# Cameronr11/GAN-Variant-Research

Hardware: AMD Instinct MI355X
Metric: images/sec (G+D train step) 256x256 CUT (higher is better)
Workload: dtype bf16; 1 GPU; CUT ResNet-9 G + PatchGAN D + PatchNCE + identity + lazy R1 + DiffAugment, 256x256, batch 16 per GPU (BASELINE.json configs[2]); global_batch=16, parallelism=dp1

## Files before the change

### gan-variant-research_amd/csrc/wgrad_patch.hip

```cpp
#include <stdlib.h>
#include <atomic>
#include "common.h"

namespace {

constexpr int KM = 128;
constexpr int NB = 128, CB = 64;
constexpr int RX = 320;
constexpr int GT_BYTES = KM * 256, XP_BYTES = RX * 128, STAGE_BYTES = GT_BYTES + XP_BYTES;
constexpr int LDS_BYTES = 2 * STAGE_BYTES;
constexpr int NT = 9;
constexpr int RING_SLOTS = 4, RING_PITCH = 136;
constexpr int LDS_BYTES_RING = 2 * GT_BYTES + RING_SLOTS * RING_PITCH * 128;

struct WpArgs {
  const char* x; const char* g; float* part;
  int B, HoWo, Wo, lgWo, spi, per;
  int ipb;
  int Cx, N, pitch, nrows;
  int x_Hp, x_Wp, x_y0, x_x0;
  int g_Hp, g_Wp, g_C, g_y0, g_x0;
  int NBLK, CBLK;
};

__device__ __forceinline__ void glds16q(const char* gbase, uint32_t goff, char* lds) {
  __builtin_amdgcn_global_load_lds((const __attribute__((address_space(1))) void*)(gbase + goff),
                                   (__attribute__((address_space(3))) void*)lds, 16, 0, 0);
}

template <bool RING>
__global__ __launch_bounds__(512) void wgrad_patch_kernel(WpArgs a) {
  extern __shared__ __attribute__((aligned(1024))) char lds[];
  const int tid = threadIdx.x, lane = tid & 63, wave = tid >> 6;

  int bid = (gridDim.x & 7) == 0 ? (int)(blockIdx.x & 7) * (int)(gridDim.x >> 3) + (int)(blockIdx.x >> 3) : (int)blockIdx.x;
  const int cb = bid % a.CBLK; bid /= a.CBLK;
  const int nb = bid % a.NBLK; bid /= a.NBLK;
  const int sp = bid;
  const int b0 = a.ipb > 1 ? sp * a.ipb : sp / a.spi, sub = a.ipb > 1 ? 0 : sp - b0 * a.spi;
  const int m_begin = sub * a.per, m_end = min(a.HoWo, m_begin + a.per);
  const int nst_img = (m_end - m_begin + KM - 1) / KM;
  const int nstage = nst_img * a.ipb;
  const int n0 = nb * NB, c0 = cb * CB;

  const int gr = tid >> 4, gp = tid & 15;
  const uint32_t gsrc = (uint32_t)((n0 + ((gp ^ ((gr & 7) << 1)) << 3)) * 2);
  const int xr = tid >> 3, xp = tid & 7;
  const uint32_t xsrc = (uint32_t)((c0 + ((((xp >> 1) ^ ((xr >> 1) & 3)) << 1 | (xp & 1)) << 3)) * 2);
  const uint32_t x_pixb = (uint32_t)a.Cx * 2u, g_pixb = (uint32_t)a.g_C * 2u;

  char* const ring = lds + 2 * GT_BYTES;
  const uint32_t ring_rowb = (uint32_t)(a.pitch * 128);
  const int b = b0;
  auto load_row = [&](int iy) {
    char* slot = ring + (uint32_t)(iy & (RING_SLOTS - 1)) * ring_rowb;
    const int iyc = iy < a.x_Hp ? iy : a.x_Hp - 1;
#pragma unroll
    for (int i = 0; i < 3; ++i) {
      const int row = xr + 64 * i;
      if (row < a.pitch) {
        int ix = row + a.x_x0;
        ix = ix < a.x_Wp ? ix : a.x_Wp - 1;
        glds16q(a.x, (uint32_t)((b * a.x_Hp + iyc) * a.x_Wp + ix) * x_pixb + xsrc, slot + wave * 1024 + i * 8192);
      }
    }
  };
  auto stage = [&](int st, int buf) {
    char* gt = lds + buf * (RING ? GT_BYTES : STAGE_BYTES);
    char* xw = gt + GT_BYTES;
    const int img = st / nst_img, b = b0 + img;
    const int m0 = m_begin + (st - img * nst_img) * KM, ho0 = m0 >> a.lgWo;
#pragma unroll
    for (int i = 0; i < 4; ++i) {
      int m = m0 + gr + 32 * i;
      m = m < a.HoWo ? m : a.HoWo - 1;
      const int ho = m >> a.lgWo, wo = m & (a.Wo - 1);
      glds16q(a.g, (uint32_t)((b * a.g_Hp + ho + a.g_y0) * a.g_Wp + wo + a.g_x0) * g_pixb + gsrc, gt + wave * 1024 + i * 8192);
    }
    if constexpr (RING) { load_row(ho0 + 2 + a.x_y0); return; }
#pragma unroll
    for (int i = 0; i < 5; ++i) {
      const int row = xr + 64 * i;
      if (row < a.nrows * a.pitch) {
        const int wr = row / a.pitch, wcol = row - wr * a.pitch;
        int iy = ho0 + wr + a.x_y0, ix = wcol + a.x_x0;
        iy = iy < a.x_Hp ? iy : a.x_Hp - 1;
        ix = ix < a.x_Wp ? ix : a.x_Wp - 1;
        glds16q(a.x, (uint32_t)((b * a.x_Hp + iy) * a.x_Wp + ix) * x_pixb + xsrc, xw + wave * 1024 + i * 8192);
      }
    }
  };

  const int wn = wave >> 2, wc = wave & 3;
  const int fr = lane & 15, fg = lane >> 4, q = fr >> 2, p4 = fr & 3;
  uint32_t gcol[4];
#pragma unroll
  for (int i = 0; i < 4; ++i) gcol[i] = (uint32_t)(((wn * 4 + i) * 16 + p4 * 4) * 2);
  const uint32_t xcol = (uint32_t)((wc * 16 + p4 * 4) * 2);
  const uint32_t rowb = (uint32_t)(a.pitch * 128);
  const int kl = 4 * fg + q;
  uint32_t gbase[4], xbase[3];
#pragma unroll
  for (int i = 0; i < 4; ++i) gbase[i] = (uint32_t)(kl * 256) + (gcol[i] ^ (uint32_t)((kl & 7) << 5));
#pragma unroll
  for (int dx = 0; dx < 3; ++dx) {
    const int r = kl + dx;
    xbase[dx] = (uint32_t)(r * 128) + (xcol ^ (uint32_t)((r & 6) << 4));
  }

  f32x4_t acc[4][NT];
#pragma unroll
  for (int i = 0; i < 4; ++i)
#pragma unroll
    for (int t = 0; t < NT; ++t) acc[i][t] = f32x4_t{0.f, 0.f, 0.f, 0.f};

  if constexpr (RING) { const int iy0 = (m_begin >> a.lgWo) + a.x_y0; load_row(iy0); load_row(iy0 + 1); }
  stage(0, 0);
  for (int st = 0; st < nstage; ++st) {
    __syncthreads();
    char* gt = lds + (st & 1) * (RING ? GT_BYTES : STAGE_BYTES);
    const char* xw = RING ? ring : gt + GT_BYTES;
    const int m0 = m_begin + (st % nst_img) * KM;
    uint32_t so[3] = {0u, 0u, 0u};
    if constexpr (RING) {
      const int iy0 = (m0 >> a.lgWo) + a.x_y0;
#pragma unroll
      for (int dy = 0; dy < 3; ++dy) so[dy] = (uint32_t)((iy0 + dy) & (RING_SLOTS - 1)) * ring_rowb;
    }
    if (m0 + KM > m_end) {
      for (int c = tid; c < KM * 16; c += 512)
        if (m0 + (c >> 4) >= m_end) *reinterpret_cast<u32x4_t*>(gt + c * 16) = u32x4_t{0, 0, 0, 0};
      __syncthreads();
    }
    if (st + 1 < nstage) stage(st + 1, (st + 1) & 1);
#pragma unroll
    for (int ks = 0; ks < KM / 32; ++ks) {
      asm volatile("" : "+v"(gbase[0]), "+v"(gbase[1]), "+v"(gbase[2]), "+v"(gbase[3]), "+v"(xbase[0]), "+v"(xbase[1]), "+v"(xbase[2]));
      s16x4_t gf[4][2];
      uint32_t xh[2][3];
#pragma unroll
      for (int h = 0; h < 2; ++h) {
        const int ku = ks * 32 + 16 * h;
        const uint32_t goff = (uint32_t)(ku * 256);
        const uint32_t xoff = RING ? (uint32_t)(ku * 128) : (uint32_t)(((ku >> a.lgWo) * a.pitch + (ku & (a.Wo - 1))) * 128);
#pragma unroll
        for (int i = 0; i < 4; ++i)
          gf[i][h] = __builtin_amdgcn_ds_read_tr16_b64_v4i16((__attribute__((address_space(3))) s16x4_t*)(gt + gbase[i] + goff));
#pragma unroll
        for (int dx = 0; dx < 3; ++dx) xh[h][dx] = xbase[dx] + xoff;
      }
      bf16x8_t av[4];
#pragma unroll
      for (int i = 0; i < 4; ++i)
        av[i] = bf16x8_t{gf[i][0][0], gf[i][0][1], gf[i][0][2], gf[i][0][3], gf[i][1][0], gf[i][1][1], gf[i][1][2], gf[i][1][3]};
      s16x4_t xf[3][2];
      auto x_read = [&](int t) {
#pragma unroll
        for (int h = 0; h < 2; ++h)
          xf[t % 3][h] = __builtin_amdgcn_ds_read_tr16_b64_v4i16(
              (__attribute__((address_space(3))) s16x4_t*)(xw + xh[h][t % 3] + (RING ? so[t / 3] : (uint32_t)(t / 3) * rowb)));
      };
      x_read(0);
      x_read(1);
#pragma unroll
      for (int t = 0; t < NT; ++t) {
        if (t + 2 < NT) x_read(t + 2);
        const bf16x8_t bv = {xf[t % 3][0][0], xf[t % 3][0][1], xf[t % 3][0][2], xf[t % 3][0][3],
                             xf[t % 3][1][0], xf[t % 3][1][1], xf[t % 3][1][2], xf[t % 3][1][3]};
#pragma unroll
        for (int i = 0; i < 4; ++i) acc[i][t] = __builtin_amdgcn_mfma_f32_16x16x32_bf16(av[i], bv, acc[i][t], 0, 0, 0);
      }
    }
  }

  float* part = a.part + (int64_t)sp * a.N * NT * a.Cx;
#pragma unroll
  for (int i = 0; i < 4; ++i)
#pragma unroll
    for (int t = 0; t < NT; ++t)
#pragma unroll
      for (int e = 0; e < 4; ++e) {
        const int n = n0 + (wn * 4 + i) * 16 + fg * 4 + e;
        part[((int64_t)n * NT + t) * a.Cx + c0 + wc * 16 + fr] = acc[i][t][e];
      }
}

}

int gan_wgrad_patch_fp8_splits(const gan_wgrad_desc* d);
int gan_wgrad_patch_fp8_launch(const gan_wgrad_desc* d, hipStream_t s);

extern "C" int gan_wgrad_patch_splits(const gan_wgrad_desc* d) {
  if (!d) return 0;
  if (d->dtype == GAN_FP8) return gan_wgrad_patch_fp8_splits(d);
  if (d->dtype != GAN_BF16 || d->ntaps != NT || d->Cx % CB != 0 || d->N % NB != 0 || d->N != d->g_C) return 0;
  if (d->x_sy != 1 || d->x_sx != 1 || d->g_sy != 1 || d->g_sx != 1) return 0;
  if (d->Wo < 16 || (d->Wo & (d->Wo - 1)) != 0 || KM % d->Wo != 0 || d->max_tapoff != (2 * d->x_Wp + 2) * d->Cx) return 0;
  const int HoWo = d->Ho * d->Wo;
  if (HoWo < KM) return 0;
  const int pitch = (d->Wo + 2 + 7) / 8 * 8, nrows = KM / d->Wo + 2;
  if (nrows * pitch > RX && !(d->Wo == KM && pitch == RING_PITCH)) return 0;
  const int blocks_per_split = (d->N / NB) * (d->Cx / CB);
  if (HoWo < 8 * KM && d->B * blocks_per_split > 256 && HoWo % KM == 0 && nrows * pitch <= RX) {
    int ipb = d->B * blocks_per_split / 256;
    while (ipb > 1 && d->B % ipb != 0) --ipb;
    if (ipb > 1) return -ipb;
  }
  if (HoWo < 8 * KM && d->B > 64) return 0;
  int spi = (256 + d->B * blocks_per_split - 1) / (d->B * blocks_per_split);
  const int max_spi = HoWo / (2 * KM) > 0 ? HoWo / (2 * KM) : 1;
  if (spi > max_spi) spi = max_spi;
  if (spi < 1) spi = 1;
  return spi;
}

int gan_wgrad_patch_launch(const gan_wgrad_desc* d, hipStream_t s) {
  if (d->dtype == GAN_FP8) return gan_wgrad_patch_fp8_launch(d, s);
  const int spi_want = gan_wgrad_patch_splits(d);
  GAN_CHECK(spi_want != 0 && d->nsplit > 0 && (d->nsplit % d->B == 0 || (d->B % d->nsplit == 0 && (d->Ho * d->Wo) % KM == 0)),
            "wgrad: variant=1 but the descriptor does not qualify for the range-patch kernel");
  WpArgs a;
  a.x = (const char*)d->x; a.g = (const char*)d->g; a.part = d->part;
  a.B = d->B; a.HoWo = d->Ho * d->Wo; a.Wo = d->Wo; a.lgWo = __builtin_ctz(d->Wo);
  a.ipb = d->nsplit < d->B ? d->B / d->nsplit : 1;
  a.spi = a.ipb > 1 ? 1 : d->nsplit / d->B;
  int per = (a.HoWo + a.spi - 1) / a.spi;
  per = (per + KM - 1) / KM * KM;
  a.per = per;
  GAN_CHECK((a.spi - 1) * per < a.HoWo, "wgrad_patch: nsplit=%d leaves empty splits", d->nsplit);
  a.Cx = d->Cx; a.N = d->N; a.pitch = (d->Wo + 2 + 7) / 8 * 8; a.nrows = KM / d->Wo + 2;
  a.x_Hp = d->x_Hp; a.x_Wp = d->x_Wp; a.x_y0 = d->x_y0; a.x_x0 = d->x_x0;
  a.g_Hp = d->g_Hp; a.g_Wp = d->g_Wp; a.g_C = d->g_C; a.g_y0 = d->g_y0; a.g_x0 = d->g_x0;
  a.NBLK = d->N / NB; a.CBLK = d->Cx / CB;
  const bool ring = a.nrows * a.pitch > RX;
  GAN_CHECK(spi_want > 0 ? d->nsplit == d->B * spi_want : d->nsplit * -spi_want == d->B, "wgrad_patch: nsplit=%d is not what gan_wgrad_patch_splits implies (%d)",
            d->nsplit, spi_want);
  GAN_CHECK(!(ring && a.ipb > 1), "wgrad_patch: the row-ring variant (128-pixel-wide maps) takes one image per split");
  GAN_CHECK((int64_t)d->B * d->x_Hp * d->x_Wp * d->Cx * 2 < (1ll << 32) && (int64_t)d->B * d->g_Hp * d->g_Wp * d->g_C * 2 < (1ll << 32),
            "wgrad_patch: an operand tensor exceeds the kernel's 32-bit byte offsets (4 GiB): split the batch");
  static std::atomic<uint64_t> attr_devs{0};
  int dev = 0;
  if (hipGetDevice(&dev) != hipSuccess) return gan_set_error(-2, "wgrad_patch: hipGetDevice failed");
  const uint64_t dev_bit = 1ull << (dev & 63);
  if (!(attr_devs.load(std::memory_order_acquire) & dev_bit)) {
    if (hipFuncSetAttribute((const void*)wgrad_patch_kernel<false>, hipFuncAttributeMaxDynamicSharedMemorySize, LDS_BYTES) != hipSuccess ||
        hipFuncSetAttribute((const void*)wgrad_patch_kernel<true>, hipFuncAttributeMaxDynamicSharedMemorySize, LDS_BYTES_RING) != hipSuccess)
      return gan_set_error(-2, "wgrad_patch: cannot raise the dynamic LDS limit to %d bytes", LDS_BYTES);
    attr_devs.fetch_or(dev_bit, std::memory_order_release);
  }
  if (a.nrows * a.pitch > RX) hipLaunchKernelGGL(wgrad_patch_kernel<true>, dim3(a.NBLK * a.CBLK * d->nsplit), dim3(512), LDS_BYTES_RING, s, a);
  else hipLaunchKernelGGL(wgrad_patch_kernel<false>, dim3(a.NBLK * a.CBLK * d->nsplit), dim3(512), LDS_BYTES, s, a);
  if (hipGetLastError() != hipSuccess) return gan_set_error(-2, "wgrad_patch: launch failed");
  return 0;
}
```

Before: 739.2 images/s.

## Unify wgrad patch kernel on a per-width row ring with explicit DMA waits

Replaces the two wgrad kernel variants (a per-stage halo window and a 4-slot row ring for 128-wide maps) with one kernel templated on log2 of the output width. It always keeps input rows in an LDS ring, so the two halo rows shared by adjacent stages are loaded once instead of reloaded. The DMA into LDS uses inline asm that sets m0, and the stage sync uses explicit vmcnt/lgkmcnt waits plus s_barrier instead of __syncthreads. The pipeline depth is a template constant, still 1 here. It adds four template instantiations and hand-written inline asm, which risks mistakes in the wait counts.

Result: faster. 759.8 images/s (median of 6 runs) (+2.8%).

```diff
diff --git a/gan-variant-research_amd/csrc/wgrad_patch.hip b/gan-variant-research_amd/csrc/wgrad_patch.hip
--- a/gan-variant-research_amd/csrc/wgrad_patch.hip
+++ b/gan-variant-research_amd/csrc/wgrad_patch.hip
@@ -6,32 +6,50 @@
 
 constexpr int KM = 128;
 constexpr int NB = 128, CB = 64;
-constexpr int RX = 320;
-constexpr int GT_BYTES = KM * 256, XP_BYTES = RX * 128, STAGE_BYTES = GT_BYTES + XP_BYTES;
-constexpr int LDS_BYTES = 2 * STAGE_BYTES;
 constexpr int NT = 9;
-constexpr int RING_SLOTS = 4, RING_PITCH = 136;
-constexpr int LDS_BYTES_RING = 2 * GT_BYTES + RING_SLOTS * RING_PITCH * 128;
+constexpr int KS = 128;
+constexpr int DEPTH = 1;
+constexpr int NGT = DEPTH + 1;
+constexpr int GS_BYTES = KS * 256;
+template <int LGWO> struct Ring {
+  static constexpr int WO = 1 << LGWO, R = KS / WO;
+  static constexpr bool MULTI = WO < KM;
+  static constexpr int PITCH = (WO + 2 + 7) / 8 * 8, ROWB = PITCH * 128, CPR = PITCH / 8;
+  static constexpr int SLOTS = (R + 2) + DEPTH * R + (MULTI ? 2 * ((DEPTH * KS + KM - 1) / KM) : 0);
+  static constexpr int X_CHUNKS = R * CPR, LEAD_CHUNKS = 2 * CPR, G_DMA = KS / 32, X_DMA = (X_CHUNKS + 7) / 8, LEAD_DMA = (LEAD_CHUNKS + 7) / 8;
+  static constexpr int DMA_PER_STAGE = G_DMA + X_DMA;
+  static constexpr int LDS = NGT * GS_BYTES + SLOTS * ROWB;
+  static_assert(KS % WO == 0 && KM % KS == 0, "a stage is whole image rows and a split is whole stages");
+  static_assert(DMA_PER_STAGE * (DEPTH - 1) < 64, "vmcnt is a 6-bit counter");
+  static_assert(R + 2 <= SLOTS && LDS <= 160 * 1024, "the ring does not fit the CU's 160 KiB of LDS");
+};
 
 struct WpArgs {
   const char* x; const char* g; float* part;
-  int B, HoWo, Wo, lgWo, spi, per;
+  int HoWo, spi, per;
   int ipb;
-  int Cx, N, pitch, nrows;
+  int Cx, N;
   int x_Hp, x_Wp, x_y0, x_x0;
   int g_Hp, g_Wp, g_C, g_y0, g_x0;
   int NBLK, CBLK;
 };
 
-__device__ __forceinline__ void glds16q(const char* gbase, uint32_t goff, char* lds) {
-  __builtin_amdgcn_global_load_lds((const __attribute__((address_space(1))) void*)(gbase + goff),
-                                   (__attribute__((address_space(3))) void*)lds, 16, 0, 0);
-}
-
-template <bool RING>
+__device__ __forceinline__ void dma16(const char* gbase, uint32_t goff, uint32_t lds_dst) {
+  uint32_t keep;
+  asm volatile("s_mov_b32 %0, m0\n\ts_mov_b32 m0, %3\n\ts_nop 0\n\tglobal_load_lds_dwordx4 %1, %2\n\ts_mov_b32 m0, %0"
+               : "=&s"(keep) : "v"(goff), "s"(gbase), "s"(__builtin_amdgcn_readfirstlane(lds_dst)) : "memory");
+}
+template <int K, int DMA_PER_STAGE> __device__ __forceinline__ void retire_and_barrier(int in_flight) {
+  if constexpr (K == 0) asm volatile("s_waitcnt vmcnt(0) lgkmcnt(0)\n\ts_barrier" ::: "memory");
+  else if (in_flight >= K) asm volatile("s_waitcnt vmcnt(%0) lgkmcnt(0)\n\ts_barrier" :: "n"(K * DMA_PER_STAGE) : "memory");
+  else retire_and_barrier<K - 1, DMA_PER_STAGE>(in_flight);
+}
+
+template <int LGWO>
 __global__ __launch_bounds__(512) void wgrad_patch_kernel(WpArgs a) {
+  using G = Ring<LGWO>;
   extern __shared__ __attribute__((aligned(1024))) char lds[];
-  const int tid = threadIdx.x, lane = tid & 63, wave = tid >> 6;
+  const int tid = threadIdx.x, lane = tid & 63, wave = __builtin_amdgcn_readfirstlane(tid >> 6);
 
   int bid = (gridDim.x & 7) == 0 ? (int)(blockIdx.x & 7) * (int)(gridDim.x >> 3) + (int)(blockIdx.x >> 3) : (int)blockIdx.x;
   const int cb = bid % a.CBLK; bid /= a.CBLK;
@@ -39,56 +57,53 @@
   const int sp = bid;
   const int b0 = a.ipb > 1 ? sp * a.ipb : sp / a.spi, sub = a.ipb > 1 ? 0 : sp - b0 * a.spi;
   const int m_begin = sub * a.per, m_end = min(a.HoWo, m_begin + a.per);
-  const int nst_img = (m_end - m_begin + KM - 1) / KM;
+  const int nst_img = (m_end - m_begin + KM - 1) / KM * (KM / KS);
   const int nstage = nst_img * a.ipb;
-  const int n0 = nb * NB, c0 = cb * CB;
+  const int n0 = nb * NB, c0 = cb * CB, ho0 = m_begin >> LGWO;
 
   const int gr = tid >> 4, gp = tid & 15;
   const uint32_t gsrc = (uint32_t)((n0 + ((gp ^ ((gr & 7) << 1)) << 3)) * 2);
-  const int xr = tid >> 3, xp = tid & 7;
+  const int xr = lane >> 3, xp = lane & 7;
   const uint32_t xsrc = (uint32_t)((c0 + ((((xp >> 1) ^ ((xr >> 1) & 3)) << 1 | (xp & 1)) << 3)) * 2);
   const uint32_t x_pixb = (uint32_t)a.Cx * 2u, g_pixb = (uint32_t)a.g_C * 2u;
 
-  char* const ring = lds + 2 * GT_BYTES;
-  const uint32_t ring_rowb = (uint32_t)(a.pitch * 128);
-  const int b = b0;
-  auto load_row = [&](int iy) {
-    char* slot = ring + (uint32_t)(iy & (RING_SLOTS - 1)) * ring_rowb;
-    const int iyc = iy < a.x_Hp ? iy : a.x_Hp - 1;
-#pragma unroll
-    for (int i = 0; i < 3; ++i) {
-      const int row = xr + 64 * i;
-      if (row < a.pitch) {
-        int ix = row + a.x_x0;
-        ix = ix < a.x_Wp ? ix : a.x_Wp - 1;
-        glds16q(a.x, (uint32_t)((b * a.x_Hp + iyc) * a.x_Wp + ix) * x_pixb + xsrc, slot + wave * 1024 + i * 8192);
-      }
-    }
+  const uint32_t lds0 = (uint32_t)(uintptr_t)(__attribute__((address_space(3))) char*)lds;
+  constexpr uint32_t XRING = NGT * GS_BYTES;
+  auto wrap = [](int s) { return s >= G::SLOTS ? s - G::SLOTS : s; };
+
+  auto x_chunk = [&](int b, int lr, int cc, int slot) {
+    int iy = ho0 + lr + a.x_y0, ix = cc * 8 + xr + a.x_x0;
+    iy = iy < a.x_Hp ? iy : a.x_Hp - 1;
+    ix = ix < a.x_Wp ? ix : a.x_Wp - 1;
+    dma16(a.x, (uint32_t)((b * a.x_Hp + iy) * a.x_Wp + ix) * x_pixb + xsrc, lds0 + XRING + (uint32_t)(slot * G::ROWB + cc * 1024));
   };
-  auto stage = [&](int st, int buf) {
-    char* gt = lds + buf * (RING ? GT_BYTES : STAGE_BYTES);
-    char* xw = gt + GT_BYTES;
-    const int img = st / nst_img, b = b0 + img;
-    const int m0 = m_begin + (st - img * nst_img) * KM, ho0 = m0 >> a.lgWo;
-#pragma unroll
-    for (int i = 0; i < 4; ++i) {
+  int l_img = 0, l_ls = 0, l_buf = 0, l_slot = 0;
+  auto issue = [&]() {
+    const int b = b0 + l_img, m0 = m_begin + l_ls * KS;
+#pragma unroll
+    for (int i = 0; i < G::G_DMA; ++i) {
       int m = m0 + gr + 32 * i;
       m = m < a.HoWo ? m : a.HoWo - 1;
-      const int ho = m >> a.lgWo, wo = m & (a.Wo - 1);
-      glds16q(a.g, (uint32_t)((b * a.g_Hp + ho + a.g_y0) * a.g_Wp + wo + a.g_x0) * g_pixb + gsrc, gt + wave * 1024 + i * 8192);
-    }
-    if constexpr (RING) { load_row(ho0 + 2 + a.x_y0); return; }
-#pragma unroll
-    for (int i = 0; i < 5; ++i) {
-      const int row = xr + 64 * i;
-      if (row < a.nrows * a.pitch) {
-        const int wr = row / a.pitch, wcol = row - wr * a.pitch;
-        int iy = ho0 + wr + a.x_y0, ix = wcol + a.x_x0;
-        iy = iy < a.x_Hp ? iy : a.x_Hp - 1;
-        ix = ix < a.x_Wp ? ix : a.x_Wp - 1;
-        glds16q(a.x, (uint32_t)((b * a.x_Hp + iy) * a.x_Wp + ix) * x_pixb + xsrc, xw + wave * 1024 + i * 8192);
-      }
-    }
+      const int ho = m >> LGWO, wo = m & (G::WO - 1);
+      dma16(a.g, (uint32_t)((b * a.g_Hp + ho + a.g_y0) * a.g_Wp + wo + a.g_x0) * g_pixb + gsrc,
+            lds0 + (uint32_t)(l_buf * GS_BYTES + wave * 1024 + i * 8192));
+    }
+#pragma unroll
+    for (int i = 0; i < G::X_DMA; ++i) {
+      const int c = min(wave + 8 * i, G::X_CHUNKS - 1), r = c / G::CPR;
+      x_chunk(b, l_ls * G::R + 2 + r, c - r * G::CPR, wrap(l_slot + 2 + r));
+    }
+    if (l_ls == 0) {
+#pragma unroll
+      for (int i = 0; i < G::LEAD_DMA; ++i) {
+        const int c = min(wave + 8 * i, G::LEAD_CHUNKS - 1), r = c / G::CPR;
+        x_chunk(b, r, c - r * G::CPR, wrap(l_slot + r));
+      }
+    }
+    l_buf = l_buf + 1 == NGT ? 0 : l_buf + 1;
+    l_slot += G::R;
+    if (++l_ls == nst_img) { l_ls = 0; ++l_img; l_slot += 2; }
+    l_slot = wrap(l_slot);
   };
 
   const int wn = wave >> 2, wc = wave & 3;
@@ -97,7 +112,6 @@
 #pragma unroll
   for (int i = 0; i < 4; ++i) gcol[i] = (uint32_t)(((wn * 4 + i) * 16 + p4 * 4) * 2);
   const uint32_t xcol = (uint32_t)((wc * 16 + p4 * 4) * 2);
-  const uint32_t rowb = (uint32_t)(a.pitch * 128);
   const int kl = 4 * fg + q;
   uint32_t gbase[4], xbase[3];
 #pragma unroll
@@ -105,7 +119,7 @@
 #pragma unroll
   for (int dx = 0; dx < 3; ++dx) {
     const int r = kl + dx;
-    xbase[dx] = (uint32_t)(r * 128) + (xcol ^ (uint32_t)((r & 6) << 4));
+    xbase[dx] = XRING + (uint32_t)(r * 128) + (xcol ^ (uint32_t)((r & 6) << 4));
   }
 
   f32x4_t acc[4][NT];
@@ -114,40 +128,31 @@
 #pragma unroll
     for (int t = 0; t < NT; ++t) acc[i][t] = f32x4_t{0.f, 0.f, 0.f, 0.f};
 
-  if constexpr (RING) { const int iy0 = (m_begin >> a.lgWo) + a.x_y0; load_row(iy0); load_row(iy0 + 1); }
-  stage(0, 0);
+  for (int s = 0; s < DEPTH && s < nstage; ++s) issue();
+  int r_ls = 0, r_buf = 0, r_slot = 0;
   for (int st = 0; st < nstage; ++st) {
-    __syncthreads();
-    char* gt = lds + (st & 1) * (RING ? GT_BYTES : STAGE_BYTES);
-    const char* xw = RING ? ring : gt + GT_BYTES;
-    const int m0 = m_begin + (st % nst_img) * KM;
-    uint32_t so[3] = {0u, 0u, 0u};
-    if constexpr (RING) {
-      const int iy0 = (m0 >> a.lgWo) + a.x_y0;
-#pragma unroll
-      for (int dy = 0; dy < 3; ++dy) so[dy] = (uint32_t)((iy0 + dy) & (RING_SLOTS - 1)) * ring_rowb;
-    }
-    if (m0 + KM > m_end) {
-      for (int c = tid; c < KM * 16; c += 512)
+    retire_and_barrier<DEPTH - 1, G::DMA_PER_STAGE>(nstage - 1 - st);
+    char* gt = lds + r_buf * GS_BYTES;
+    const int m0 = m_begin + r_ls * KS;
+    uint32_t so[G::R + 2];
+#pragma unroll
+    for (int j = 0; j < G::R + 2; ++j) so[j] = (uint32_t)(wrap(r_slot + j) * G::ROWB);
+    if (m0 + KS > m_end) {
+      for (int c = tid; c < KS * 16; c += 512)
         if (m0 + (c >> 4) >= m_end) *reinterpret_cast<u32x4_t*>(gt + c * 16) = u32x4_t{0, 0, 0, 0};
-      __syncthreads();
-    }
-    if (st + 1 < nstage) stage(st + 1, (st + 1) & 1);
-#pragma unroll
-    for (int ks = 0; ks < KM / 32; ++ks) {
+      asm volatile("s_waitcnt lgkmcnt(0)\n\ts_barrier" ::: "memory");
+    }
+    if (st + DEPTH < nstage) issue();
+#pragma unroll
+    for (int ks = 0; ks < KS / 32; ++ks) {
       asm volatile("" : "+v"(gbase[0]), "+v"(gbase[1]), "+v"(gbase[2]), "+v"(gbase[3]), "+v"(xbase[0]), "+v"(xbase[1]), "+v"(xbase[2]));
       s16x4_t gf[4][2];
-      uint32_t xh[2][3];
 #pragma unroll
       for (int h = 0; h < 2; ++h) {
-        const int ku = ks * 32 + 16 * h;
-        const uint32_t goff = (uint32_t)(ku * 256);
-        const uint32_t xoff = RING ? (uint32_t)(ku * 128) : (uint32_t)(((ku >> a.lgWo) * a.pitch + (ku & (a.Wo - 1))) * 128);
+        const uint32_t goff = (uint32_t)((ks * 32 + 16 * h) * 256);
 #pragma unroll
         for (int i = 0; i < 4; ++i)
           gf[i][h] = __builtin_amdgcn_ds_read_tr16_b64_v4i16((__attribute__((address_space(3))) s16x4_t*)(gt + gbase[i] + goff));
-#pragma unroll
-        for (int dx = 0; dx < 3; ++dx) xh[h][dx] = xbase[dx] + xoff;
       }
       bf16x8_t av[4];
 #pragma unroll
@@ -156,9 +161,11 @@
       s16x4_t xf[3][2];
       auto x_read = [&](int t) {
 #pragma unroll
-        for (int h = 0; h < 2; ++h)
+        for (int h = 0; h < 2; ++h) {
+          const int ku = ks * 32 + 16 * h;
           xf[t % 3][h] = __builtin_amdgcn_ds_read_tr16_b64_v4i16(
-              (__attribute__((address_space(3))) s16x4_t*)(xw + xh[h][t % 3] + (RING ? so[t / 3] : (uint32_t)(t / 3) * rowb)));
+              (__attribute__((address_space(3))) s16x4_t*)(lds + (xbase[t % 3] + so[(ku >> LGWO) + t / 3]) + (ku & (G::WO - 1)) * 128));
+        }
       };
       x_read(0);
       x_read(1);
@@ -171,6 +178,10 @@
         for (int i = 0; i < 4; ++i) acc[i][t] = __builtin_amdgcn_mfma_f32_16x16x32_bf16(av[i], bv, acc[i][t], 0, 0, 0);
       }
     }
+    r_buf = r_buf + 1 == NGT ? 0 : r_buf + 1;
+    r_slot += G::R;
+    if (++r_ls == nst_img) { r_ls = 0; r_slot += 2; }
+    r_slot = wrap(r_slot);
   }
 
   float* part = a.part + (int64_t)sp * a.N * NT * a.Cx;
@@ -183,6 +194,20 @@
         const int n = n0 + (wn * 4 + i) * 16 + fg * 4 + e;
         part[((int64_t)n * NT + t) * a.Cx + c0 + wc * 16 + fr] = acc[i][t][e];
       }
+}
+
+template <int LGWO> int launch_ring(const WpArgs& a, int nsplit, hipStream_t s) {
+  static std::atomic<uint64_t> attr_devs{0};
+  int dev = 0;
+  if (hipGetDevice(&dev) != hipSuccess) return gan_set_error(-2, "wgrad_patch: hipGetDevice failed");
+  const uint64_t dev_bit = 1ull << (dev & 63);
+  if (!(attr_devs.load(std::memory_order_acquire) & dev_bit)) {
+    if (hipFuncSetAttribute((const void*)wgrad_patch_kernel<LGWO>, hipFuncAttributeMaxDynamicSharedMemorySize, Ring<LGWO>::LDS) != hipSuccess)
+      return gan_set_error(-2, "wgrad_patch: cannot raise the dynamic LDS limit to %d bytes", Ring<LGWO>::LDS);
+    attr_devs.fetch_or(dev_bit, std::memory_order_release);
+  }
+  hipLaunchKernelGGL(wgrad_patch_kernel<LGWO>, dim3(a.NBLK * a.CBLK * nsplit), dim3(512), Ring<LGWO>::LDS, s, a);
+  return 0;
 }
 
 }
@@ -198,10 +223,8 @@
   if (d->Wo < 16 || (d->Wo & (d->Wo - 1)) != 0 || KM % d->Wo != 0 || d->max_tapoff != (2 * d->x_Wp + 2) * d->Cx) return 0;
   const int HoWo = d->Ho * d->Wo;
   if (HoWo < KM) return 0;
-  const int pitch = (d->Wo + 2 + 7) / 8 * 8, nrows = KM / d->Wo + 2;
-  if (nrows * pitch > RX && !(d->Wo == KM && pitch == RING_PITCH)) return 0;
   const int blocks_per_split = (d->N / NB) * (d->Cx / CB);
-  if (HoWo < 8 * KM && d->B * blocks_per_split > 256 && HoWo % KM == 0 && nrows * pitch <= RX) {
+  if (HoWo < 8 * KM && d->B * blocks_per_split > 256 && HoWo % KM == 0 && d->Wo < KM) {
     int ipb = d->B * blocks_per_split / 256;
     while (ipb > 1 && d->B % ipb != 0) --ipb;
     if (ipb > 1) return -ipb;
@@ -221,35 +244,26 @@
             "wgrad: variant=1 but the descriptor does not qualify for the range-patch kernel");
   WpArgs a;
   a.x = (const char*)d->x; a.g = (const char*)d->g; a.part = d->part;
-  a.B = d->B; a.HoWo = d->Ho * d->Wo; a.Wo = d->Wo; a.lgWo = __builtin_ctz(d->Wo);
+  a.HoWo = d->Ho * d->Wo;
   a.ipb = d->nsplit < d->B ? d->B / d->nsplit : 1;
   a.spi = a.ipb > 1 ? 1 : d->nsplit / d->B;
   int per = (a.HoWo + a.spi - 1) / a.spi;
   per = (per + KM - 1) / KM * KM;
   a.per = per;
   GAN_CHECK((a.spi - 1) * per < a.HoWo, "wgrad_patch: nsplit=%d leaves empty splits", d->nsplit);
-  a.Cx = d->Cx; a.N = d->N; a.pitch = (d->Wo + 2 + 7) / 8 * 8; a.nrows = KM / d->Wo + 2;
+  a.Cx = d->Cx; a.N = d->N;
   a.x_Hp = d->x_Hp; a.x_Wp = d->x_Wp; a.x_y0 = d->x_y0; a.x_x0 = d->x_x0;
   a.g_Hp = d->g_Hp; a.g_Wp = d->g_Wp; a.g_C = d->g_C; a.g_y0 = d->g_y0; a.g_x0 = d->g_x0;
   a.NBLK = d->N / NB; a.CBLK = d->Cx / CB;
-  const bool ring = a.nrows * a.pitch > RX;
   GAN_CHECK(spi_want > 0 ? d->nsplit == d->B * spi_want : d->nsplit * -spi_want == d->B, "wgrad_patch: nsplit=%d is not what gan_wgrad_patch_splits implies (%d)",
             d->nsplit, spi_want);
-  GAN_CHECK(!(ring && a.ipb > 1), "wgrad_patch: the row-ring variant (128-pixel-wide maps) takes one image per split");
+  GAN_CHECK(!(d->Wo == KM && a.ipb > 1), "wgrad_patch: 128-pixel-wide maps take one image per split");
   GAN_CHECK((int64_t)d->B * d->x_Hp * d->x_Wp * d->Cx * 2 < (1ll << 32) && (int64_t)d->B * d->g_Hp * d->g_Wp * d->g_C * 2 < (1ll << 32),
             "wgrad_patch: an operand tensor exceeds the kernel's 32-bit byte offsets (4 GiB): split the batch");
-  static std::atomic<uint64_t> attr_devs{0};
-  int dev = 0;
-  if (hipGetDevice(&dev) != hipSuccess) return gan_set_error(-2, "wgrad_patch: hipGetDevice failed");
-  const uint64_t dev_bit = 1ull << (dev & 63);
-  if (!(attr_devs.load(std::memory_order_acquire) & dev_bit)) {
-    if (hipFuncSetAttribute((const void*)wgrad_patch_kernel<false>, hipFuncAttributeMaxDynamicSharedMemorySize, LDS_BYTES) != hipSuccess ||
-        hipFuncSetAttribute((const void*)wgrad_patch_kernel<true>, hipFuncAttributeMaxDynamicSharedMemorySize, LDS_BYTES_RING) != hipSuccess)
-      return gan_set_error(-2, "wgrad_patch: cannot raise the dynamic LDS limit to %d bytes", LDS_BYTES);
-    attr_devs.fetch_or(dev_bit, std::memory_order_release);
-  }
-  if (a.nrows * a.pitch > RX) hipLaunchKernelGGL(wgrad_patch_kernel<true>, dim3(a.NBLK * a.CBLK * d->nsplit), dim3(512), LDS_BYTES_RING, s, a);
-  else hipLaunchKernelGGL(wgrad_patch_kernel<false>, dim3(a.NBLK * a.CBLK * d->nsplit), dim3(512), LDS_BYTES, s, a);
+  const int lgWo = __builtin_ctz(d->Wo);
+  const int rc = lgWo == 4 ? launch_ring<4>(a, d->nsplit, s) : lgWo == 5 ? launch_ring<5>(a, d->nsplit, s)
+               : lgWo == 6 ? launch_ring<6>(a, d->nsplit, s) : launch_ring<7>(a, d->nsplit, s);
+  if (rc != 0) return rc;
   if (hipGetLastError() != hipSuccess) return gan_set_error(-2, "wgrad_patch: launch failed");
   return 0;
 }
```
